# kit-cel/vae-equalizer

Measured on AMD Instinct MI355X. Metric: equalized symbols/s/GPU, DP 64-QAM VAE-LE, higher is better.
Workload: dtype f32

## Files before the change

vae_equalizer_amd/csrc/vaeq_dp_wave_kernel.h:

```cpp
#pragma once
#include <hip/hip_runtime.h>
#include <stdint.h>
#include <type_traits>

#include "vaeq.h"
#include "vaeq_common.h"
#include "vaeq_launch.h"
#include "vaeq_wave.h"

#ifdef VAEQ_PHASE_STAMPS
#define VAEQ_STAMP(i) do { if (s == a.steps - 1) tst[i] = __builtin_readcyclecounter(); } while (0)
#define VAEQ_XSTAMP(i) do { if (s == a.steps - 1) tsx[i] = __builtin_readcyclecounter(); } while (0)
#else
#define VAEQ_STAMP(i) do { } while (0)
#define VAEQ_XSTAMP(i) do { } while (0)
#endif
#define VAEQ_NSTAMP 12
#ifndef VAEQ_PIPE
#define VAEQ_PIPE 1
#endif
#define VAEQ_BT_FRAMES 16
#ifndef VAEQ_WPS
#define VAEQ_WPS 2
#endif

namespace vaeq {

__device__ __forceinline__ float half_sum(float a0, float a1)
{
    const auto r = __builtin_amdgcn_permlane32_swap(__builtin_bit_cast(unsigned, a0), __builtin_bit_cast(unsigned, a1), false, false);
    return __builtin_bit_cast(float, (unsigned)r[0]) + __builtin_bit_cast(float, (unsigned)r[1]);
}

struct WaveLayout {
    int Lph, Uph;
    int X, E, U, PSv, W, H, PSh, VS, MOM, RED, XG, total;
};

__host__ __device__ inline WaveLayout wave_layout(int B, int M, int NW = 1)
{
    WaveLayout l;
    const int len = 2 * B + M - 1;
    const int lph = wave_lph(len);
    l.Lph = lph;
    l.Uph = B / 2 + 1;
    int o = 0;
    auto take = [&](int bytes) { int r = o; o += (bytes + 15) & ~15; return r; };
    l.X = take(2 * 4 * lph * 8);
    l.E = take(2 * 4 * lph * 8);
    const int ubytes = 2 * 2 * l.Uph * 8, gbytes = 2 * B * 8;
    l.U = take(ubytes > gbytes ? ubytes : gbytes);
    l.PSv = take(2 * (B + 1) * 4);
    l.W = take(2 * M * 16);
    l.H = take(2 * 2 * (M + 1) * 8);
    l.PSh = take(2 * (M + 1) * 4);
    l.VS = take(2 * M * 4);
    l.MOM = take(16 * 64 * 4);
    l.RED = take(NW > 1 ? 64 * 4 : 0);
    l.XG = take((NW - 1) * 4 * 64 * 4);
    l.total = o;
    return l;
}

template <int M, bool INIT, bool PIPE = true, bool SPLIT = true>
__device__ __forceinline__ void pair_fir(cacc (&acc)[2][2], cacc (&accx)[2][2], const float2 *xp, int Lph, const float4 *wq)
{
    cacc (&acc2)[2][2] = SPLIT ? accx : acc;
    auto tapA = [&](int k) -> v2f { return lds2(reinterpret_cast<const float2 *>(wq + k)); };
    auto tapB = [&](int k) -> v2f { return lds2(reinterpret_cast<const float2 *>(wq + k) + 1); };
    constexpr int G = M / 4;
    auto load = [&](int g, v2f (&r)[14]) {
        const float2 *xg = xp + g;
        r[0] = lds2(xg); r[1] = lds2(xg + Lph); r[2] = lds2(xg + 2 * Lph); r[3] = lds2(xg + 3 * Lph); r[4] = lds2(xg + 1); r[5] = lds2(xg + Lph + 1);
#pragma unroll
        for (int t = 0; t < 4; t++) { r[6 + 2 * t] = tapA(4 * g + t); r[7 + 2 * t] = tapB(4 * g + t); }
    };
    auto fma = [&](int, const v2f (&r)[14], auto first) {
        constexpr bool F = decltype(first)::value;
        cmacf<F>(acc[0][0], r[6], r[0]); cmacf<F>(acc[0][1], r[7], r[0]); cmacf<F>(acc[1][0], r[6], r[2]); cmacf<F>(acc[1][1], r[7], r[2]);
        cmacf<F && SPLIT>(acc2[0][0], r[8], r[1]); cmacf<F && SPLIT>(acc2[0][1], r[9], r[1]);
        cmacf<F && SPLIT>(acc2[1][0], r[8], r[3]); cmacf<F && SPLIT>(acc2[1][1], r[9], r[3]);
        cmac(acc[0][0], r[10], r[2]); cmac(acc[0][1], r[11], r[2]); cmac(acc[1][0], r[10], r[4]); cmac(acc[1][1], r[11], r[4]);
        cmac(acc2[0][0], r[12], r[3]); cmac(acc2[0][1], r[13], r[3]); cmac(acc2[1][0], r[12], r[5]); cmac(acc2[1][1], r[13], r[5]);
    };
    pipe2<14, INIT, PIPE>(G, load, fma);
#pragma unroll
    for (int k = 4 * G; k < M; k++) {
        const v2f a = tapA(k), b = tapB(k);
        const v2f xa = lds2(xp + (k & 3) * Lph + (k >> 2)), xb = lds2(xp + ((k + 2) & 3) * Lph + ((k + 2) >> 2));
        if (k & 1) { cmac(acc2[0][0], a, xa); cmac(acc2[0][1], b, xa); cmac(acc2[1][0], a, xb); cmac(acc2[1][1], b, xb); }
        else { cmac(acc[0][0], a, xa); cmac(acc[0][1], b, xa); cmac(acc[1][0], a, xb); cmac(acc[1][1], b, xb); }
    }
}

template <int M, bool MERGE = true>
__device__ __forceinline__ void pair_du(cacc (&acc)[2][2][2], const float2 *ep, int Lph, const float2 *ht, int MP)
{
    constexpr int G = M / 4;
    auto load1 = [&](int chi, int g, v2f *x) {
        const float2 *xg = ep + chi * 4 * Lph + g;
        x[0] = lds2(xg); x[1] = lds2(xg + Lph); x[2] = lds2(xg + 2 * Lph); x[3] = lds2(xg + 3 * Lph); x[4] = lds2(xg + 1); x[5] = lds2(xg + Lph + 1);
#pragma unroll
        for (int t = 0; t < 4; t++) { x[6 + 2 * t] = lds2(ht + (chi * 2 + 0) * MP + 4 * g + t); x[7 + 2 * t] = lds2(ht + (chi * 2 + 1) * MP + 4 * g + t); }
    };
    auto fma1 = [&](int chi, const v2f *x, int t, auto first) {
        constexpr bool F = decltype(first)::value;
        cmacf<F>(acc[chi][0][0], x[6 + 2 * t], x[t]); cmacf<F>(acc[chi][0][1], x[7 + 2 * t], x[t]);
        cmacf<F>(acc[chi][1][0], x[6 + 2 * t], x[t + 2]); cmacf<F>(acc[chi][1][1], x[7 + 2 * t], x[t + 2]);
    };
    if constexpr (MERGE) {
        auto load = [&](int g, v2f (&r)[28]) { load1(0, g, r); load1(1, g, r + 14); };
        auto fma = [&](int, const v2f (&r)[28], auto first) {
            fma1(0, r, 0, first); fma1(1, r + 14, 0, first);
#pragma unroll
            for (int t = 1; t < 4; t++) { fma1(0, r, t, std::false_type{}); fma1(1, r + 14, t, std::false_type{}); }
        };
        pipe2<28, true, false>(G, load, fma);
    } else {
#pragma unroll
        for (int chi = 0; chi < 2; chi++) {
            auto load = [&](int g, v2f (&r)[14]) { load1(chi, g, r); };
            auto fma = [&](int, const v2f (&r)[14], auto first) {
                fma1(chi, r, 0, first);
#pragma unroll
                for (int t = 1; t < 4; t++) fma1(chi, r, t, std::false_type{});
            };
            pipe2<14, true, false>(G, load, fma);
        }
    }
#pragma unroll
    for (int k = 4 * G; k < M; k++)
#pragma unroll
        for (int chi = 0; chi < 2; chi++) {
            const float2 *xp = ep + chi * 4 * Lph;
            const v2f a = lds2(ht + (chi * 2 + 0) * MP + k), b = lds2(ht + (chi * 2 + 1) * MP + k);
            const v2f xa = lds2(xp + (k & 3) * Lph + (k >> 2)), xb = lds2(xp + ((k + 2) & 3) * Lph + ((k + 2) >> 2));
            cmac(acc[chi][0][0], a, xa); cmac(acc[chi][0][1], b, xa); cmac(acc[chi][1][0], a, xb); cmac(acc[chi][1][1], b, xb);
        }
}

constexpr bool uniform_parts(int B, int M, int NP)
{
    const int mh = M / 2, nm = 2 * B - 2 * mh;
    for (int par = 0; par < 2; par++) {
        const int T = (nm - par + 1) >> 1, Th = ((T + 2 * NP - 1) / (2 * NP)) << 1;
        int n0 = -1;
        for (int part = 0; part < NP; part++) {
            const int ma = (part * Th) >> 1, e = part * Th + Th, mb = ((T < e ? T : e) + 1) >> 1;
            if (mb - ma <= 0 || (n0 >= 0 && mb - ma != n0)) return false;
            n0 = mb - ma;
        }
    }
    const int Bq = ((B + 2 * NP - 1) / (2 * NP)) << 1;
    int n0 = -1;
    for (int part = 0; part < NP; part++) {
        const int ma = (part * Bq) >> 1, e = part * Bq + Bq, mb = (B < e ? B : e) >> 1;
        if (mb - ma <= 0 || (n0 >= 0 && mb - ma != n0)) return false;
        n0 = mb - ma;
    }
    return true;
}

template <int M, int NLEV, int BT, bool PAIR, int OUT, int NW = 1, int BL = 0>
__global__ __launch_bounds__(64 * NW, VAEQ_WPS) void dp_wave_kernel(const vaeq_dp_args a)
{
    constexpr int mh = M / 2, Mh = 2 * mh, MP = M + 1;
    constexpr float LOG2E = 1.4426950408889634f, LN2 = 0.6931471805599453f;
    extern __shared__ float4 smem4[];
    char *sm = reinterpret_cast<char *>(smem4);
    const int gl = threadIdx.x, lane = NW > 1 ? (gl & 63) : gl, wv = NW > 1 ? (gl >> 6) : 0, run = blockIdx.x;
    constexpr int NT = 64 * NW, NP = 2 * NW;
    constexpr bool UNI = BT > 0 && uniform_parts(BT, M, NP);
    constexpr bool FIXL = BT > 0 || (BL > 0 && M != 13 && M != 17 && !(M == 31 && NW == 1));
    constexpr bool PIPE = VAEQ_PIPE && FIXL;
    constexpr bool WIDE = FIXL;
    constexpr bool B100 = BT == 100 && NW == 1;
    constexpr int QAUX = B100 ? 2 : 0;
    const int B = BT ? BT : a.B;
    const int BS = BT ? BT : BL ? BL : B;
    constexpr bool ODDB = BT == 0 && BL > 0;
    const int L = 2 * B, nm = L - Mh, P2 = ODDB ? (B + 1) / 2 : B / 2;
    const float rnm = 1.0f / (float)nm;
    const WaveLayout lay = wave_layout(BS, M, NW);
    const int Lph = lay.Lph, Uph = lay.Uph;
    float2 *Xs = reinterpret_cast<float2 *>(sm + lay.X), *Es = reinterpret_cast<float2 *>(sm + lay.E);
    float2 *Us = reinterpret_cast<float2 *>(sm + lay.U), *GY = Us;
    float4 *Wt = reinterpret_cast<float4 *>(sm + lay.W);
    float2 *Ht = reinterpret_cast<float2 *>(sm + lay.H);
    float *PSv = reinterpret_cast<float *>(sm + lay.PSv);
    float *PSh = reinterpret_cast<float *>(sm + lay.PSh);
    float *VS = reinterpret_cast<float *>(sm + lay.VS);
    float *RED = reinterpret_cast<float *>(sm + lay.RED), *XG = reinterpret_cast<float *>(sm + lay.XG);

    float amp[NLEV], b2[NLEV], nlogP[NLEV];
    const float nusc = a.nu_sc[run];
#pragma unroll
    for (int i = 0; i < NLEV; i++) {
        amp[i] = a.amp[i];
        b2[i] = nusc * amp[i] * amp[i] * LOG2E;
        nlogP[i] = -logf(a.P[(size_t)run * NLEV + i]);
    }
    const float var0 = a.var[run * 2 + 0], var1 = a.var[run * 2 + 1];
    const float lrW = a.lr_W[run], lrH = a.lr_h[run];

    for (int i = gl; i < (lay.W - lay.X) / 8; i += NT) Xs[i] = make_float2(0.f, 0.f);
    for (int i = gl; i < (lay.PSh - lay.H) / 8; i += NT) Ht[i] = make_float2(0.f, 0.f);
    __syncthreads();
    const int tk = lane & 31, half = lane >> 5;
    const bool worker = tk < M, owner = worker && wv == 0;
    const int part = wv * 2 + half;
    const size_t gbase = (size_t)run * 8 * M;
    float *MOM = reinterpret_cast<float *>(sm + lay.MOM) + lane;
#define mWr(p) MOM[(0 + (p)) * 64]
#define mWi(p) MOM[(2 + (p)) * 64]
#define vWr(p) MOM[(4 + (p)) * 64]
#define vWi(p) MOM[(6 + (p)) * 64]
#define mHr(p) MOM[(8 + (p)) * 64]
#define mHi(p) MOM[(10 + (p)) * 64]
#define vHr(p) MOM[(12 + (p)) * 64]
#define vHi(p) MOM[(14 + (p)) * 64]
    if (owner) {
#pragma unroll
        for (int p = 0; p < 2; p++) {
            const size_t ir = gbase + (half * 4 + p) * M + tk, ii = gbase + (half * 4 + 2 + p) * M + tk;
            float *wq = reinterpret_cast<float *>(&Wt[p * M + tk]);
            wq[half * 2 + 0] = a.W[ir];
            wq[half * 2 + 1] = a.W[ii];
            mWr(p) = a.adam_mW[ir]; mWi(p) = a.adam_mW[ii];
            vWr(p) = a.adam_vW[ir]; vWi(p) = a.adam_vW[ii];
            const size_t hr = gbase + ((half * 2 + p) * 2 + 0) * M + tk, hi = hr + M;
            Ht[(half * 2 + p) * MP + tk] = make_float2(a.h[hr], a.h[hi]);
            mHr(p) = a.adam_mh[hr]; mHi(p) = a.adam_mh[hi];
            vHr(p) = a.adam_vh[hr]; vHi(p) = a.adam_vh[hi];
        }
    }
    int step = a.step[run];
    __shared__ double BTW[2][VAEQ_BT_FRAMES];
    if (gl < VAEQ_BT_FRAMES && gl < a.n_frames) {
        const double t = (double)(step + gl * a.steps);
        BTW[0][gl] = pow(0.9, t);
        BTW[1][gl] = pow(0.999, t);
    }
    __syncthreads();
    double b1t = BTW[0][0], b2t = BTW[1][0];

    const int klen = a.keep_len, k0 = a.keep_off;
    const size_t No = (size_t)a.steps * klen;
    constexpr bool pairst = PAIR;
    const bool act = gl < P2;
    const int nq = (nm + 3) / 4;
    const int n0 = 2 * gl;
    const bool v1 = ODDB ? act && (n0 + 1 < B) : act;
    const float2 *Xl = Xs + gl, *El = Es + gl, *Ul = Us + gl;
    const float2 *Xa = Xs + (act ? gl : 0), *Ea = Es + (act ? gl : 0);

    const bool ldl = gl < (ODDB ? (L + 3) / 4 : L / 4);
    float4 pf[4];
    const uint32_t S4 = (uint32_t)a.S * 4u;
    auto frame_rsrc = [&](int f) { return make_rsrc(a.rx + ((size_t)run * a.n_frames + f) * 4 * (size_t)a.S, 4u * S4); };
    auto fetch = [&](const __amdgpu_buffer_rsrc_t xr, int s) {
        const uint32_t vo = ldl ? ((uint32_t)s * (uint32_t)a.stride_sym * 2u + 4u * gl) * 4u : OOB;
#pragma unroll
        for (int r = 0; r < 4; r++) pf[r] = bld128(xr, vo, (uint32_t)r * S4);
    };
#ifdef VAEQ_PHASE_STAMPS
    long long tst[VAEQ_NSTAMP], tsx[8];
#endif
    fetch(frame_rsrc(0), 0);
    for (int f = 0; f < a.n_frames; f++) {
        const __amdgpu_buffer_rsrc_t xr = frame_rsrc(f), xn = frame_rsrc(f + 1 < a.n_frames ? f + 1 : f);
        if (f && f < VAEQ_BT_FRAMES) {
            b1t = BTW[0][f];
            b2t = BTW[1][f];
        }
        const bool qf = OUT != 2 && a.q_out, yf = a.y_out, ef = OUT != 1 && a.eq_out, df = OUT != 1 && a.dec_out;
        const uint32_t No4 = (uint32_t)No * 4u;
        const size_t fr = (size_t)run * a.n_frames + f;
        const __amdgpu_buffer_rsrc_t qr = make_rsrc(qf ? a.q_out + fr * (4 * NLEV) * No : nullptr, qf ? 4u * NLEV * No4 : 0u);
        const __amdgpu_buffer_rsrc_t yr = make_rsrc(yf ? a.y_out + fr * 4 * No : nullptr, yf ? 4u * No4 : 0u);
        const __amdgpu_buffer_rsrc_t er = make_rsrc(ef ? a.eq_out + fr * 2 * No : nullptr, ef ? 2u * No4 : 0u);
        const __amdgpu_buffer_rsrc_t dr = make_rsrc(df ? a.dec_out + fr * 4 * No : nullptr, df ? (uint32_t)(4 * No) : 0u);
        const __amdgpu_buffer_rsrc_t lr_ = make_rsrc(a.loss ? a.loss + fr * a.steps : nullptr, a.loss ? (uint32_t)a.steps * 4u : 0u);
        const __amdgpu_buffer_rsrc_t vr_ = make_rsrc(a.var_est ? a.var_est + fr * 2 * a.steps : nullptr, a.var_est ? (uint32_t)a.steps * 8u : 0u);
#pragma unroll 1
        for (int s = 0; s < a.steps; s++) {
            VAEQ_STAMP(0);
            if (ldl) {
#pragma unroll
                for (int p = 0; p < 2; p++) {
                    const float4 I4 = pf[p * 2 + 0], Q4 = pf[p * 2 + 1];
                    const float xi[4] = {I4.x, I4.y, I4.z, I4.w}, xq[4] = {Q4.x, Q4.y, Q4.z, Q4.w};
#pragma unroll
                    for (int i = 0; i < 4; i++) {
                        const int c = mh + i;
                        const bool in = !ODDB || 4 * gl + i < L;
                        Xs[(p * 4 + (c & 3)) * Lph + gl + (c >> 2)] = in ? make_float2(xi[i], xq[i]) : make_float2(0.f, 0.f);
                    }
                }
            }
            sync_lds<NW>();

            VAEQ_STAMP(1);
            float2 y[2][2];
            {
                cacc ya[2][2], yb[2][2];
                pair_fir<M, true, PIPE, WIDE>(ya, yb, Xa, Lph, Wt);
                pair_fir<M, false, PIPE, WIDE>(ya, yb, Xa + 4 * Lph, Lph, Wt + M);
#pragma unroll
                for (int sy = 0; sy < 2; sy++)
#pragma unroll
                    for (int o = 0; o < 2; o++) {
                        if constexpr (WIDE) {
                            ya[sy][o].a += yb[sy][o].a;
                            ya[sy][o].b += yb[sy][o].b;
                        }
                        y[sy][o] = cfin(ya[sy][o]);
                    }
            }
            asm volatile("" : "+v"(y[0][0].x), "+v"(y[0][0].y), "+v"(y[0][1].x), "+v"(y[0][1].y), "+v"(y[1][0].x), "+v"(y[1][0].y),
                         "+v"(y[1][1].x), "+v"(y[1][1].y));
            VAEQ_STAMP(2);
            const bool kept0 = act && (n0 >= k0) && (n0 < k0 + klen), kept1 = act && (n0 + 1 >= k0) && (n0 + 1 < k0 + klen);
            const uint32_t col = (uint32_t)(s * klen + (n0 - k0));
            const uint32_t vo0 = kept0 ? col * 4u : OOB, vo1 = kept1 ? col * 4u + 4u : OOB;
            if (yf) {
                uint32_t yrow = 0u;
                auto next_row = [&]() {
                    yrow += No4;
                    asm volatile("" : "+s"(yrow));
                };
#pragma unroll
                for (int o = 0; o < 2; o++) {
                    const uint32_t r0 = yrow;
                    next_row();
                    const uint32_t r1 = yrow;
                    next_row();
                    if (pairst) {
                        bst64(v2f{y[0][o].x, y[1][o].x}, yr, vo0, r0);
                        bst64(v2f{y[0][o].y, y[1][o].y}, yr, vo0, r1);
                    } else {
                        bst32(y[0][o].x, yr, vo0, r0); bst32(y[0][o].y, yr, vo0, r1);
                        bst32(y[1][o].x, yr, vo1, r0); bst32(y[1][o].y, yr, vo1, r1);
                    }
                }
            }

            VAEQ_STAMP(3);
            float mv[2][2][2], mt3[2][2][2], mkc[2][2][2];
            uint32_t qrow = 0u;
            float klsum = 0.f, vv[2][2];
#pragma unroll
            for (int o = 0; o < 2; o++) {
                const float c2 = 0.5f / (o ? var1 : var0) * LOG2E;
                float2 muv[2];
#pragma unroll
                for (int c = 0; c < 2; c++) {
                    const v2f yy = c ? v2f{y[0][o].y, y[1][o].y} : v2f{y[0][o].x, y[1][o].x};
                    v2f z[NLEV], q[NLEV];
                    v2f ssum = {0.f, 0.f};
                    float zm0 = -3.0e38f, zm1 = -3.0e38f;
#pragma unroll
                    for (int i = 0; i < NLEV; i++) {
                        const v2f d = yy - amp[i];
                        z[i] = -(d * d * c2 + b2[i]);
                        zm0 = fmaxf(zm0, z[i].x);
                        zm1 = fmaxf(zm1, z[i].y);
                    }
                    const v2f zmax = {zm0, zm1};
#pragma unroll
                    for (int i = 0; i < NLEV; i++) {
                        z[i] -= zmax;
                        q[i] = v2f{__builtin_amdgcn_exp2f(z[i].x), __builtin_amdgcn_exp2f(z[i].y)};
                        ssum += q[i];
                    }
                    const v2f rs = {__builtin_amdgcn_rcpf(ssum.x), __builtin_amdgcn_rcpf(ssum.y)};
                    v2f m1 = {0.f, 0.f};
#pragma unroll
                    for (int i = 0; i < NLEV; i++) {
                        q[i] *= rs;
                        m1 += q[i] * amp[i];
                    }
                    if (ef && c == 0) {
                        if (pairst) bst64(m1, er, vo0, (uint32_t)o * No4);
                        else { bst32(m1.x, er, vo0, (uint32_t)o * No4); bst32(m1.y, er, vo1, (uint32_t)o * No4); }
                    }
                    if (df) {
                        float v0 = q[0].x, v1 = q[0].y;
                        int b0 = 0, b1 = 0;
#pragma unroll
                        for (int i = 1; i < NLEV; i++) {
                            if (q[i].x > v0) { v0 = q[i].x; b0 = i; }
                            if (q[i].y > v1) { v1 = q[i].y; b1 = i; }
                        }
                        const uint32_t ro = (uint32_t)(o * 2 + c) * (uint32_t)No;
                        if (pairst) bst16((unsigned short)(b0 | (b1 << 8)), dr, kept0 ? col : OOB, ro);
                        else { bst8((unsigned char)b0, dr, kept0 ? col : OOB, ro); bst8((unsigned char)b1, dr, kept1 ? col + 1u : OOB, ro); }
                    }
                    v2f m2 = {0.f, 0.f}, m3 = {0.f, 0.f}, kk = {0.f, 0.f}, kl = {0.f, 0.f};
#pragma unroll
                    for (int i = 0; i < NLEV; i++) {
                        const v2f d = amp[i] - m1, qd = q[i] * d, g = z[i] * LN2 + nlogP[i];
                        m2 += qd * d;
                        m3 += qd * d * d;
                        kk += qd * g;
                        kl += q[i] * g;
                    }
                    const bool inr0 = (n0 >= mh) && (n0 < B - mh) && act;
                    const bool inr1 = (n0 + 1 >= mh) && (n0 + 1 < B - mh) && act;
                    if (inr0) klsum += kl.x - __builtin_amdgcn_logf(ssum.x) * LN2;
                    if (inr1) klsum += kl.y - __builtin_amdgcn_logf(ssum.y) * LN2;
                    asm volatile("" : "+v"(m2), "+v"(m3), "+v"(kk), "+v"(klsum));
                    mv[0][o][c] = m2.x; mv[1][o][c] = m2.y;
                    mt3[0][o][c] = m3.x; mt3[1][o][c] = m3.y;
                    mkc[0][o][c] = inr0 ? kk.x : 0.f;
                    mkc[1][o][c] = inr1 ? kk.y : 0.f;
                    if (c) { muv[0].y = m1.x; muv[1].y = m1.y; } else { muv[0].x = m1.x; muv[1].x = m1.y; }
                    if (qf) {
#pragma unroll
                        for (int i = 0; i < NLEV; i++) {
                            const uint32_t ro = qrow;
                            if (pairst) bst64<QAUX>(q[i], qr, vo0, ro);
                            else { bst32<QAUX>(q[i].x, qr, vo0, ro); bst32<QAUX>(q[i].y, qr, vo1, ro); }
                            qrow += No4;
                            asm volatile("" : "+s"(qrow));
                        }
                    }
                }
                vv[o][0] = act ? mv[0][o][0] + mv[0][o][1] : 0.f;
                vv[o][1] = v1 ? mv[1][o][0] + mv[1][o][1] : 0.f;
                if (act) {
                    Us[(o * 2 + 0) * Uph + gl] = muv[0];
                    Us[(o * 2 + 1) * Uph + gl] = v1 ? muv[1] : make_float2(0.f, 0.f);
                }
            }
            VAEQ_STAMP(4);
            {
                float inc[2];
#pragma unroll
                for (int o = 0; o < 2; o++) inc[o] = wave_incl_scan_dpp(vv[o][0] + vv[o][1]);
                if constexpr (NW > 1) {
                    if (lane == 63) { RED[wv] = inc[0]; RED[NW + wv] = inc[1]; }
                    sync_lds<NW>();
#pragma unroll
                    for (int w = 0; w < NW - 1; w++)
                        if (w < wv) { inc[0] += RED[w]; inc[1] += RED[NW + w]; }
                }
#pragma unroll
                for (int o = 0; o < 2; o++) {
                    if (act) {
                        PSv[o * (BS + 1) + n0 + 1] = inc[o] - vv[o][1];
                        PSv[o * (BS + 1) + n0 + 2] = inc[o];
                    }
                    if (gl == 0) PSv[o * (BS + 1)] = 0.f;
                }
            }
            sync_lds<NW>();
            if (owner) {
                const int lo = (Mh - tk + 1) >> 1, hi_ = (nm - 1 + Mh - tk) >> 1;
                VS[half * M + tk] = PSv[half * (BS + 1) + hi_ + 1] - PSv[half * (BS + 1) + lo];
            }
            sync_lds<NW>();

            VAEQ_STAMP(5);
            float se0 = 0.f, se1 = 0.f;
            float hq0 = 0.f, hq1 = 0.f;
            if (worker) {
                const float2 h0 = Ht[(0 * 2 + half) * MP + tk], h1 = Ht[(1 * 2 + half) * MP + tk];
                hq0 = h0.x * h0.x + h0.y * h0.y;
                hq1 = h1.x * h1.x + h1.y * h1.y;
            }
            const float vsl = worker ? VS[half * M + tk] : 0.f;
            {
                cacc D[2][4];
                constexpr int NA = mh + 1, NB = NA / 2;
#pragma unroll
                for (int v = 0; v < 2; v++) {
                    const float2 *h0 = Ht + (0 * 2 + v) * MP, *h1 = Ht + (1 * 2 + v) * MP;
                    const float2 *up = Us + (gl < nq ? gl : 0) + v * 2 * Uph;
                    auto step_a = [&](int aa, v2f ulo, v2f uhi, auto first) {
                        constexpr bool F = decltype(first)::value;
                        const v2f e0 = lds2(h0 + 2 * aa), o0 = lds2(h0 + 2 * aa + 1), e1 = lds2(h1 + 2 * aa), o1 = lds2(h1 + 2 * aa + 1);
                        cmacf<F>(D[0][0], e0, ulo); cmacf<F>(D[0][1], o0, ulo);
                        cmacf<F>(D[0][2], e0, uhi); cmacf<F>(D[0][3], o0, uhi);
                        cmacf<F>(D[1][0], e1, ulo); cmacf<F>(D[1][1], o1, ulo);
                        cmacf<F>(D[1][2], e1, uhi); cmacf<F>(D[1][3], o1, uhi);
                    };
                    if (NA & 1) {
                        if (v == 0) step_a(mh, lds2(up), lds2(up + Uph), std::true_type{});
                        else step_a(mh, lds2(up), lds2(up + Uph), std::false_type{});
                    } else if (v == 0) {
#pragma unroll
                        for (int chi = 0; chi < 2; chi++)
#pragma unroll
                            for (int i = 0; i < 4; i++) D[chi][i] = cacc0();
                    }
                    constexpr int ph = mh & 1;
                    auto load = [&](int b, v2f (&r)[11]) {
                        const int sl = (mh >> 1) - b;
                        r[0] = lds2(up + ph * Uph + sl);
                        r[1] = lds2(up + (ph ^ 1) * Uph + sl + ph);
                        r[2] = lds2(up + (ph ^ 1) * Uph + sl + ph - 1);
#pragma unroll
                        for (int t = 0; t < 4; t++) { r[3 + t] = lds2(h0 + 4 * b + t); r[7 + t] = lds2(h1 + 4 * b + t); }
                    };
                    auto fma = [&](int, const v2f (&r)[11], auto) {
                        cmac(D[0][0], r[3], r[0]); cmac(D[0][1], r[4], r[0]); cmac(D[0][2], r[3], r[1]); cmac(D[0][3], r[4], r[1]);
                        cmac(D[1][0], r[7], r[0]); cmac(D[1][1], r[8], r[0]); cmac(D[1][2], r[7], r[1]); cmac(D[1][3], r[8], r[1]);
                        cmac(D[0][0], r[5], r[2]); cmac(D[0][1], r[6], r[2]); cmac(D[0][2], r[5], r[0]); cmac(D[0][3], r[6], r[0]);
                        cmac(D[1][0], r[9], r[2]); cmac(D[1][1], r[10], r[2]); cmac(D[1][2], r[9], r[0]); cmac(D[1][3], r[10], r[0]);
                    };
                    pipe2<11, false, PIPE>(NB, load, fma);
                }
                VAEQ_STAMP(6);
                if (gl < nq) {
#pragma unroll
                    for (int chi = 0; chi < 2; chi++)
#pragma unroll
                        for (int i = 0; i < 4; i++) {
                            const int ce = Mh + i;
                            const float2 x = Xl[(chi * 4 + (ce & 3)) * Lph + (ce >> 2)];
                            const float2 Dv = cfin(D[chi][i]);
                            float2 e = make_float2(x.x - Dv.x, x.y - Dv.y);
                            if (4 * gl + i >= nm) e = make_float2(0.f, 0.f);
                            Es[(chi * 4 + (ce & 3)) * Lph + gl + (ce >> 2)] = e;
                            const float e2 = e.x * e.x + e.y * e.y;
                            if (chi) se1 += e2; else se0 += e2;
                        }
                }
            }
            se0 = wave_sum_dpp(se0);
            se1 = wave_sum_dpp(se1);
            klsum = wave_sum_dpp(klsum);
            if constexpr (NW > 1) {
                if (lane == 0) { RED[16 + wv] = se0; RED[16 + NW + wv] = se1; RED[16 + 2 * NW + wv] = klsum; }
                sync_lds<NW>();
                se0 = RED[16]; se1 = RED[16 + NW]; klsum = RED[16 + 2 * NW];
#pragma unroll
                for (int w = 1; w < NW; w++) { se0 += RED[16 + w]; se1 += RED[16 + NW + w]; klsum += RED[16 + 2 * NW + w]; }
            }
            const float C0 = se0 + wave_sum_dpp(hq0 * vsl), C1 = se1 + wave_sum_dpp(hq1 * vsl);
            const float gC0 = (float)nm * __builtin_amdgcn_rcpf(C0), gC1 = (float)nm * __builtin_amdgcn_rcpf(C1);
            {
                const uint32_t vo = gl == 0 ? 0u : OOB;
                if (a.loss) bst32((float)nm * LN2 * (__builtin_amdgcn_logf(C0) + __builtin_amdgcn_logf(C1)) + klsum, lr_, vo, (uint32_t)s * 4u);
                if (a.var_est) {
                    bst32(C0 * rnm, vr_, vo, (uint32_t)s * 4u);
                    bst32(C1 * rnm, vr_, vo, ((uint32_t)a.steps + (uint32_t)s) * 4u);
                }
            }
            {
                const float inc = half_incl_scan_dpp(gC0 * hq0 + gC1 * hq1);
                if (owner) PSh[half * MP + tk + 1] = inc;
                if (tk == 0) PSh[half * MP] = 0.f;
            }
            sync_lds<NW>();

            VAEQ_STAMP(7);
            step += 1;
            b1t *= 0.9;
            b2t *= 0.999;
            const float rbc1 = __builtin_amdgcn_rcpf((float)(1.0 - b1t));
            const float bc2s = __builtin_amdgcn_rcpf(__builtin_amdgcn_sqrtf((float)(1.0 - b2t)));
            const float ssW = lrW * rbc1, ssH = lrH * rbc1;
            float2 hnew[2];
            hnew[0] = hnew[1] = make_float2(0.f, 0.f);
            float ghr[2] = {0, 0}, ghi[2] = {0, 0};
            float2 hacc[2];
            {
                float2 ph_h[2] = {make_float2(0.f, 0.f), make_float2(0.f, 0.f)};
                float ph_vs[2] = {0.f, 0.f};
                if (NW == 1 && owner) {
#pragma unroll
                    for (int v = 0; v < 2; v++) {
                        ph_h[v] = Ht[(half * 2 + v) * MP + tk];
                        ph_vs[v] = VS[v * M + tk];
                    }
                }
                cacc ca[2][2];
                {
                    const int tkc = worker ? tk : 0, par = tkc & 1, aa = tkc >> 1;
                    const int T = (nm - par + 1) >> 1, Th = ((T + 2 * NP - 1) / (2 * NP)) << 1;
                    const int ma = (part * Th) >> 1, mb = (min(T, part * Th + Th) + 1) >> 1;
                    const int ceA = par + Mh, ceB = par + Mh + 2, npA = mh - aa, npB = mh - aa + 1;
                    const float2 *eA = Es + (ceA & 3) * Lph + (ceA >> 2) + ma, *eB = Es + (ceB & 3) * Lph + (ceB >> 2) + ma;
                    const float2 *uA = Us + (npA & 1) * Uph + (npA >> 1) + ma, *uB = Us + (npB & 1) * Uph + (npB >> 1) + ma;
                    auto load1 = [&](int m, v2f *r) {
                        r[0] = lds2(eA + m); r[1] = lds2(eA + 4 * Lph + m); r[2] = lds2(uA + m); r[3] = lds2(uA + 2 * Uph + m);
                        r[4] = lds2(eB + m); r[5] = lds2(eB + 4 * Lph + m); r[6] = lds2(uB + m); r[7] = lds2(uB + 2 * Uph + m);
                    };
                    cacc cbx[2][2];
                    cacc (&cb)[2][2] = WIDE ? cbx : ca;
                    auto fma1 = [&](const v2f *r, auto first) {
                        constexpr bool F = decltype(first)::value;
                        cmacf<F>(ca[0][0], r[2], r[0]); cmacf<F>(ca[0][1], r[3], r[0]); cmacf<F>(ca[1][0], r[2], r[1]); cmacf<F>(ca[1][1], r[3], r[1]);
                        cmacf<F && WIDE>(cb[0][0], r[6], r[4]); cmacf<F && WIDE>(cb[0][1], r[7], r[4]); cmacf<F && WIDE>(cb[1][0], r[6], r[5]); cmacf<F && WIDE>(cb[1][1], r[7], r[5]);
                    };
                    auto load = [&](int i, v2f (&r)[16]) { load1(2 * i, r); load1(2 * i + 1, r + 8); };
                    auto fma = [&](int, const v2f (&r)[16], auto first) { fma1(r, first); fma1(r + 8, std::false_type{}); };
                    int n = mb - ma;
                    VAEQ_XSTAMP(0);
                    if constexpr (UNI) {
                        n = __builtin_amdgcn_readfirstlane(n);
                        pipe2<16, true, PIPE>(n >> 1, load, fma);
                    } else {
                        ca[0][0] = ca[0][1] = ca[1][0] = ca[1][1] = cbx[0][0] = cbx[0][1] = cbx[1][0] = cbx[1][1] = cacc0();
                        pipe2<16, false, PIPE>(n >> 1, load, fma);
                    }
                    if (n & 1) {
                        v2f r[8];
                        load1(n - 1, r);
                        fma1(r, std::false_type{});
                    }
                    if constexpr (WIDE) {
#pragma unroll
                        for (int i = 0; i < 2; i++)
#pragma unroll
                            for (int j = 0; j < 2; j++) { ca[i][j].a += cbx[i][j].a; ca[i][j].b += cbx[i][j].b; }
                    }
                }
                VAEQ_XSTAMP(1);
                float2 acc[2][2];
#pragma unroll
                for (int chi = 0; chi < 2; chi++)
#pragma unroll
                    for (int v = 0; v < 2; v++) acc[chi][v] = cfinc(ca[chi][v]);
                if constexpr (B100) {
#pragma unroll
                    for (int v = 0; v < 2; v++) {
                        acc[0][v].x = acc[1][v].x = half_sum(acc[0][v].x, acc[1][v].x);
                        acc[0][v].y = acc[1][v].y = half_sum(acc[0][v].y, acc[1][v].y);
                    }
                } else {
#pragma unroll
                    for (int chi = 0; chi < 2; chi++)
#pragma unroll
                        for (int v = 0; v < 2; v++) {
                            acc[chi][v].x += __shfl_xor(acc[chi][v].x, 32, 64);
                            acc[chi][v].y += __shfl_xor(acc[chi][v].y, 32, 64);
                        }
                }
                if constexpr (NW > 1) {
#pragma unroll
                    for (int v = 0; v < 2; v++) {
                        hacc[v] = half ? acc[1][v] : acc[0][v];
                        if (wv > 0) {
                            XG[((wv - 1) * 4 + 2 * v + 0) * 64 + lane] = hacc[v].x;
                            XG[((wv - 1) * 4 + 2 * v + 1) * 64 + lane] = hacc[v].y;
                        }
                    }
                }
                VAEQ_XSTAMP(2);
                if (NW == 1 && owner) {
                    const float g = half ? gC1 : gC0;
#pragma unroll
                    for (int v = 0; v < 2; v++) {
                        const float2 ac = half ? acc[1][v] : acc[0][v];
                        const float2 hh = ph_h[v];
                        const float vs = ph_vs[v];
                        ghr[v] = g * (-2.0f * ac.x + 2.0f * hh.x * vs);
                        ghi[v] = g * (-2.0f * ac.y + 2.0f * hh.y * vs);
                        hnew[v] = hh;
                        if (!a.no_update) {
                            adam_update_fast(hnew[v].x, mHr(v), vHr(v), ghr[v], ssH, bc2s);
                            adam_update_fast(hnew[v].y, mHi(v), vHi(v), ghi[v], ssH, bc2s);
                        }
                    }
                }
            }

            asm volatile("" : "+v"(hnew[0].x), "+v"(hnew[0].y), "+v"(hnew[1].x), "+v"(hnew[1].y), "+v"(ghr[0]), "+v"(ghr[1]), "+v"(ghi[0]),
                         "+v"(ghi[1]));
            {
                const bool last_s = s + 1 == a.steps;
                if constexpr (B100) {
                    const bool more = !(last_s && f + 1 == a.n_frames);
                    const uint32_t vo = ldl && more ? ((uint32_t)(last_s ? 0 : s + 1) * (uint32_t)a.stride_sym * 2u + 4u * gl) * 4u : OOB;
#pragma unroll
                    for (int r = 0; r < 4; r++) pf[r] = bld128(last_s ? xn : xr, vo, (uint32_t)r * S4);
                } else if (!(last_s && f + 1 == a.n_frames)) fetch(last_s ? xn : xr, last_s ? 0 : s + 1);
            }
            VAEQ_XSTAMP(3);
            VAEQ_STAMP(8);
            float2 gy[2][2];
            {
                float2 au0[2][2], au1[2][2];
                {
                    cacc cu[2][2][2];
                    pair_du<M, WIDE>(cu, Ea, Lph, Ht, MP);
#pragma unroll
                    for (int sy = 0; sy < 2; sy++)
#pragma unroll
                        for (int v = 0; v < 2; v++) { au0[sy][v] = cfinc(cu[0][sy][v]); au1[sy][v] = cfinc(cu[1][sy][v]); }
                }
#pragma unroll
                for (int sy = 0; sy < 2; sy++) {
                    const int sx = 2 * (n0 + sy);
                    const int jlo = max(0, Mh - sx), jhi = max(jlo - 1, min(Mh, nm - 1 + Mh - sx));
#pragma unroll
                    for (int v = 0; v < 2; v++) {
                        const float ur = -2.0f * (gC0 * au0[sy][v].x + gC1 * au1[sy][v].x);
                        const float ui = -2.0f * (gC0 * au0[sy][v].y + gC1 * au1[sy][v].y);
                        const float gv = PSh[v * MP + jhi + 1] - PSh[v * MP + jlo];
                        const float iv = 1.0f / (v ? var1 : var0);
                        gy[sy][v].x = iv * (ur * mv[sy][v][0] + gv * mt3[sy][v][0] + mkc[sy][v][0]);
                        gy[sy][v].y = iv * (ui * mv[sy][v][1] + gv * mt3[sy][v][1] + mkc[sy][v][1]);
                    }
                }
            }
            VAEQ_STAMP(9);
            sync_lds<NW>();
            if constexpr (NW > 1) {
                if (owner) {
                    const float g = half ? gC1 : gC0;
#pragma unroll
                    for (int v = 0; v < 2; v++) {
                        float2 ac = hacc[v];
#pragma unroll
                        for (int w = 0; w < NW - 1; w++) {
                            ac.x += XG[(w * 4 + 2 * v + 0) * 64 + lane];
                            ac.y += XG[(w * 4 + 2 * v + 1) * 64 + lane];
                        }
                        const float2 hh = Ht[(half * 2 + v) * MP + tk];
                        const float vs = VS[v * M + tk];
                        ghr[v] = g * (-2.0f * ac.x + 2.0f * hh.x * vs);
                        ghi[v] = g * (-2.0f * ac.y + 2.0f * hh.y * vs);
                        hnew[v] = hh;
                        if (!a.no_update) {
                            adam_update_fast(hnew[v].x, mHr(v), vHr(v), ghr[v], ssH, bc2s);
                            adam_update_fast(hnew[v].y, mHi(v), vHi(v), ghi[v], ssH, bc2s);
                        }
                    }
                }
            }
            if (act) {
#pragma unroll
                for (int v = 0; v < 2; v++) {
                    GY[v * BS + n0] = gy[0][v];
                    GY[v * BS + n0 + 1] = v1 ? gy[1][v] : make_float2(0.f, 0.f);
                }
            }
            if (owner && !a.no_update) {
                Ht[(half * 2 + 0) * MP + tk] = hnew[0];
                Ht[(half * 2 + 1) * MP + tk] = hnew[1];
            }
            sync_lds<NW>();

            VAEQ_STAMP(10);
            float gwr[2] = {0, 0}, gwi[2] = {0, 0};
            {
                float pw_w[2][2] = {{0.f, 0.f}, {0.f, 0.f}}, pw_m[2][2] = {{0.f, 0.f}, {0.f, 0.f}}, pw_v[2][2] = {{0.f, 0.f}, {0.f, 0.f}};
                if (owner) {
#pragma unroll
                    for (int p = 0; p < 2; p++) {
                        const float *wq = reinterpret_cast<const float *>(&Wt[p * M + tk]) + half * 2;
                        pw_w[p][0] = wq[0]; pw_w[p][1] = wq[1];
                        pw_m[p][0] = mWr(p); pw_m[p][1] = mWi(p);
                        pw_v[p][0] = vWr(p); pw_v[p][1] = vWi(p);
                    }
                }
                cacc ca[2][2];
                {
                    const int tkc = worker ? tk : 0;
                    const int Be = ODDB ? B + (B & 1) : B;
                    const int Bq = ((Be + 2 * NP - 1) / (2 * NP)) << 1;
                    const int ma = (part * Bq) >> 1, mb = min(Be, part * Bq + Bq) >> 1;
                    const int cA = tkc, cB = tkc + 2;
                    const float2 *xA = Xs + (cA & 3) * Lph + (cA >> 2) + ma, *xB = Xs + (cB & 3) * Lph + (cB >> 2) + ma;
                    const float2 *G0 = GY + 2 * ma, *G1 = GY + BS + 2 * ma;
                    auto load1 = [&](int m, v2f *r) {
                        r[0] = lds2(G0 + 2 * m); r[1] = lds2(G0 + 2 * m + 1); r[2] = lds2(G1 + 2 * m); r[3] = lds2(G1 + 2 * m + 1);
                        r[4] = lds2(xA + m); r[5] = lds2(xA + 4 * Lph + m); r[6] = lds2(xB + m); r[7] = lds2(xB + 4 * Lph + m);
                    };
                    cacc cbx[2][2];
                    cacc (&cb)[2][2] = WIDE ? cbx : ca;
                    auto fma1 = [&](const v2f *r, auto first) {
                        constexpr bool F = decltype(first)::value;
                        cmacf<F>(ca[0][0], r[4], r[0]); cmacf<F>(ca[0][1], r[5], r[0]); cmacf<F>(ca[1][0], r[4], r[2]); cmacf<F>(ca[1][1], r[5], r[2]);
                        cmacf<F && WIDE>(cb[0][0], r[6], r[1]); cmacf<F && WIDE>(cb[0][1], r[7], r[1]); cmacf<F && WIDE>(cb[1][0], r[6], r[3]); cmacf<F && WIDE>(cb[1][1], r[7], r[3]);
                    };
                    auto load = [&](int i, v2f (&r)[16]) { load1(2 * i, r); load1(2 * i + 1, r + 8); };
                    auto fma = [&](int, const v2f (&r)[16], auto first) { fma1(r, first); fma1(r + 8, std::false_type{}); };
                    int n = mb - ma;
                    VAEQ_XSTAMP(4);
                    if constexpr (UNI) {
                        n = __builtin_amdgcn_readfirstlane(n);
                        pipe2<16, true, PIPE>(n >> 1, load, fma);
                    } else {
                        ca[0][0] = ca[0][1] = ca[1][0] = ca[1][1] = cbx[0][0] = cbx[0][1] = cbx[1][0] = cbx[1][1] = cacc0();
                        pipe2<16, false, PIPE>(n >> 1, load, fma);
                    }
                    if (n & 1) {
                        v2f r[8];
                        load1(n - 1, r);
                        fma1(r, std::false_type{});
                    }
                    if constexpr (WIDE) {
#pragma unroll
                        for (int i = 0; i < 2; i++)
#pragma unroll
                            for (int j = 0; j < 2; j++) { ca[i][j].a += cbx[i][j].a; ca[i][j].b += cbx[i][j].b; }
                    }
                }
                VAEQ_XSTAMP(5);
                float2 acc[2][2];
#pragma unroll
                for (int o = 0; o < 2; o++)
#pragma unroll
                    for (int pp = 0; pp < 2; pp++) acc[o][pp] = cfinc(ca[o][pp]);
                if constexpr (B100) {
#pragma unroll
                    for (int p = 0; p < 2; p++) {
                        acc[0][p].x = acc[1][p].x = half_sum(acc[0][p].x, acc[1][p].x);
                        acc[0][p].y = acc[1][p].y = half_sum(acc[0][p].y, acc[1][p].y);
                    }
                } else {
#pragma unroll
                    for (int o = 0; o < 2; o++)
#pragma unroll
                        for (int p = 0; p < 2; p++) {
                            acc[o][p].x += __shfl_xor(acc[o][p].x, 32, 64);
                            acc[o][p].y += __shfl_xor(acc[o][p].y, 32, 64);
                        }
                }
                if constexpr (NW > 1) {
#pragma unroll
                    for (int p = 0; p < 2; p++) {
                        const float2 ac = half ? acc[1][p] : acc[0][p];
                        if (wv > 0) {
                            XG[((wv - 1) * 4 + 2 * p + 0) * 64 + lane] = ac.x;
                            XG[((wv - 1) * 4 + 2 * p + 1) * 64 + lane] = ac.y;
                        }
                    }
                    sync_lds<NW>();
                }
                VAEQ_XSTAMP(6);
                if (owner) {
#pragma unroll
                    for (int p = 0; p < 2; p++) {
                        float2 ac = half ? acc[1][p] : acc[0][p];
                        if constexpr (NW > 1) {
#pragma unroll
                            for (int w = 0; w < NW - 1; w++) {
                                ac.x += XG[(w * 4 + 2 * p + 0) * 64 + lane];
                                ac.y += XG[(w * 4 + 2 * p + 1) * 64 + lane];
                            }
                        }
                        gwr[p] = ac.x;
                        gwi[p] = ac.y;
                        if (!a.no_update) {
                            float *wq = reinterpret_cast<float *>(&Wt[p * M + tk]) + half * 2;
                            float wr = pw_w[p][0], wi = pw_w[p][1];
                            adam_update_fast(wr, pw_m[p][0], pw_v[p][0], gwr[p], ssW, bc2s);
                            adam_update_fast(wi, pw_m[p][1], pw_v[p][1], gwi[p], ssW, bc2s);
                            wq[0] = wr;
                            wq[1] = wi;
                            mWr(p) = pw_m[p][0]; mWi(p) = pw_m[p][1];
                            vWr(p) = pw_v[p][0]; vWi(p) = pw_v[p][1];
                        }
                    }
                }
            }
            if (a.dbg_gW && owner && f == a.n_frames - 1 && s == a.steps - 1) {
#pragma unroll
                for (int p = 0; p < 2; p++) {
                    a.dbg_gW[gbase + (half * 4 + p) * M + tk] = gwr[p];
                    a.dbg_gW[gbase + (half * 4 + 2 + p) * M + tk] = gwi[p];
                    a.dbg_gh[gbase + ((half * 2 + p) * 2 + 0) * M + tk] = ghr[p];
                    a.dbg_gh[gbase + ((half * 2 + p) * 2 + 1) * M + tk] = ghi[p];
                }
            }
            sync_lds<NW>();
            VAEQ_XSTAMP(7);
            VAEQ_STAMP(11);
        }
    }
#ifdef VAEQ_PHASE_STAMPS
    if (gl == 0 && run == (int)gridDim.x / 2 && a.loss)
        for (int i = 0; i + 1 < VAEQ_NSTAMP; i++) a.loss[i] = (float)(tst[i + 1] - tst[i]);
    if (gl == 0 && run == (int)gridDim.x / 2 && a.loss)
        for (int i = 0; i < 7; i++) a.loss[16 + i] = (float)(tsx[i + 1] - tsx[i]);
#endif

    if (owner && !a.no_update) {
#pragma unroll
        for (int p = 0; p < 2; p++) {
            const size_t ir = gbase + (half * 4 + p) * M + tk, ii = gbase + (half * 4 + 2 + p) * M + tk;
            const float *wq = reinterpret_cast<const float *>(&Wt[p * M + tk]) + half * 2;
            a.W[ir] = wq[0]; a.W[ii] = wq[1];
            a.adam_mW[ir] = mWr(p); a.adam_mW[ii] = mWi(p);
            a.adam_vW[ir] = vWr(p); a.adam_vW[ii] = vWi(p);
            const size_t hr = gbase + ((half * 2 + p) * 2 + 0) * M + tk, hi = hr + M;
            const float2 hh = Ht[(half * 2 + p) * MP + tk];
            a.h[hr] = hh.x; a.h[hi] = hh.y;
            a.adam_mh[hr] = mHr(p); a.adam_mh[hi] = mHi(p);
            a.adam_vh[hr] = vHr(p); a.adam_vh[hi] = vHi(p);
        }
    }
    if (gl == 0 && !a.no_update) a.step[run] = step;
#undef mWr
#undef mWi
#undef vWr
#undef vWi
#undef mHr
#undef mHi
#undef vHr
#undef vHi
}


template <int M, int NLEV, int BT, int NW, int BL, bool SPEC>
static int launch_wave(const vaeq_dp_args &a, hipStream_t st)
{
    const size_t lds = (size_t)wave_layout(BL ? BL : a.B, M, NW).total;
    const bool pair = ((a.keep_len | a.keep_off) & 1) == 0;
    const int out = !SPEC ? 0 : (!a.eq_out && !a.dec_out) ? 1 : !a.q_out ? 2 : 0;
    constexpr int O1 = SPEC ? 1 : 0, O2 = SPEC ? 2 : 0;
    void (*const k[2][3])(const vaeq_dp_args) = {
        {dp_wave_kernel<M, NLEV, BT, false, 0, NW, BL>, dp_wave_kernel<M, NLEV, BT, false, O1, NW, BL>, dp_wave_kernel<M, NLEV, BT, false, O2, NW, BL>},
        {dp_wave_kernel<M, NLEV, BT, true, 0, NW, BL>, dp_wave_kernel<M, NLEV, BT, true, O1, NW, BL>, dp_wave_kernel<M, NLEV, BT, true, O2, NW, BL>}};
    note_kernel("vaeq::dp_wave_kernel<%d, %d, %d, %s, %d, %d, %d>", M, NLEV, BT, pair ? "true" : "false", out, NW, BL);
    return launch(k[pair][out], dim3(a.R), dim3(64 * NW), lds, st, a);
}

template <int M, int NLEV, int BT, int NW, int BL>
static int64_t wave_resident(int B)
{
    int nb = 0, dev = 0;
    hipDeviceProp_t prop;
    if (hipGetDevice(&dev) != hipSuccess || hipGetDeviceProperties(&prop, dev) != hipSuccess) return VAEQ_ERR_DEVICE;
    auto k = dp_wave_kernel<M, NLEV, BT, true, 0, NW, BL>;
    if (hipOccupancyMaxActiveBlocksPerMultiprocessor(&nb, k, 64 * NW, (size_t)wave_layout(BL ? BL : B, M, NW).total) != hipSuccess) return VAEQ_ERR_DEVICE;
    return (int64_t)nb * prop.multiProcessorCount;
}

template <int M, int BT, int NW>
static int launch_wave_lev(const vaeq_dp_args &a, hipStream_t st)
{
    return dispatch_nlev(a.n_lev, [&](auto nl) { return launch_wave<M, decltype(nl)::value, BT, NW, 0, (BT > 0)>(a, st); });
}
template <int M, int BT, int NW>
static int64_t wave_resident_lev(int B, int n_lev)
{
    return dispatch_nlev(n_lev, [&](auto nl) { return wave_resident<M, decltype(nl)::value, BT, NW, 0>(B); });
}
template <int M, int BL, int NW, bool SPEC>
static int launch_wave_fixl_lev(const vaeq_dp_args &a, hipStream_t st)
{
    return dispatch_nlev(a.n_lev, [&](auto nl) { return launch_wave<M, decltype(nl)::value, 0, NW, BL, SPEC>(a, st); });
}
template <int M, int BL, int NW>
static int64_t wave_resident_fixl_lev(int n_lev)
{
    return dispatch_nlev(n_lev, [&](auto nl) { return wave_resident<M, decltype(nl)::value, 0, NW, BL>(BL); });
}

template <int NW>
static int launch_wave_any(const vaeq_dp_args &a, hipStream_t st)
{
    switch (a.M) {
    case 25: return launch_wave_lev<25, 0, NW>(a, st);
    case 31: return launch_wave_fixl_lev<31, 128 * NW, NW, false>(a, st);
    case 21: return launch_wave_fixl_lev<21, 128 * NW, NW, false>(a, st);
    case 17: return launch_wave_fixl_lev<17, 128 * NW, NW, false>(a, st);
    case 13: return launch_wave_fixl_lev<13, 128 * NW, NW, false>(a, st);
    case 9: return launch_wave_fixl_lev<9, 128 * NW, NW, false>(a, st);
    }
    return VAEQ_ERR_SHAPE;
}

template <int NW>
static int64_t wave_resident_any(int B, int M, int n_lev)
{
    switch (M) {
    case 25: return wave_resident_lev<25, 0, NW>(B, n_lev);
    case 31: return wave_resident_fixl_lev<31, 128 * NW, NW>(n_lev);
    case 21: return wave_resident_fixl_lev<21, 128 * NW, NW>(n_lev);
    case 17: return wave_resident_fixl_lev<17, 128 * NW, NW>(n_lev);
    case 13: return wave_resident_fixl_lev<13, 128 * NW, NW>(n_lev);
    case 9: return wave_resident_fixl_lev<9, 128 * NW, NW>(n_lev);
    }
    return VAEQ_ERR_SHAPE;
}

}
```

Baseline: 10.52 billion.

## Map three output taus per lane in B=100 M=25 DP conv-error stage

Adds a specialized path for B=100, M=25 in which each lane computes three consecutive output positions for one polarization, with a compile-time check that the mapping covers every tau exactly once. Channel taps are loaded once and reused across the three outputs, and loads are software-pipelined. Error values go to LDS and are then re-read to form the squared-error sums. The intent is to reduce redundant LDS loads and idle lanes compared with the generic two-output mapping, at the cost of more registers and extra code complexity.

New measurement: 10.78 billion, median of 6. 1.02x the previous value.

```diff
diff --git a/vae_equalizer_amd/csrc/vaeq_dp_wave_kernel.h b/vae_equalizer_amd/csrc/vaeq_dp_wave_kernel.h
--- a/vae_equalizer_amd/csrc/vaeq_dp_wave_kernel.h
+++ b/vae_equalizer_amd/csrc/vaeq_dp_wave_kernel.h
@@ -160,6 +160,35 @@
     }
     return true;
 }
+
+struct D3Map {
+    static constexpr int TPL = 3;
+    static constexpr int nm_lanes(int T) { return (T + TPL - 1) / TPL; }
+    static constexpr int chi(int lane) { return lane >> 5; }
+    static constexpr bool works(int lane, int T) { return (lane & 31) < nm_lanes(T); }
+    static constexpr int m(int lane, int T) { return works(lane, T) ? (lane & 31) : 0; }
+    static constexpr bool stores(int lane, int i, int T) { return works(lane, T) && TPL * m(lane, T) + i < T; }
+    static constexpr bool exact(int B, int M)
+    {
+        const int mh = M / 2, T = B - mh, Uph = B / 2 + 1;
+        if (nm_lanes(T) > 32 || T > 128) return false;
+        for (int c = 0; c < 2; c++) {
+            int cnt[128] = {};
+            for (int lane = 0; lane < 64; lane++)
+                for (int i = 0; i < TPL; i++) {
+                    const int tau = TPL * m(lane, T) + i;
+                    if (tau + mh >= 2 * Uph) return false;
+                    if (chi(lane) != c || !stores(lane, i, T)) continue;
+                    if (tau >= T) return false;
+                    cnt[tau]++;
+                }
+            for (int tau = 0; tau < 128; tau++)
+                if (cnt[tau] != (tau < T ? 1 : 0)) return false;
+        }
+        return true;
+    }
+};
+static_assert(D3Map::exact(100, 25), "B = 100: three tau per lane must cover tau = 0..87 of both chi exactly once");
 
 template <int M, int NLEV, int BT, bool PAIR, int OUT, int NW = 1, int BL = 0>
 __global__ __launch_bounds__(64 * NW, VAEQ_WPS) void dp_wave_kernel(const vaeq_dp_args a)
@@ -470,7 +499,94 @@
                 hq1 = h1.x * h1.x + h1.y * h1.y;
             }
             const float vsl = worker ? VS[half * M + tk] : 0.f;
-            {
+            if constexpr (B100 && M == 25) {
+                constexpr int T = 100 - mh, NB = (mh + 1) / 2;
+                static_assert((mh & 1) == 0 && (Mh & 3) == 0 && D3Map::exact(100, M), "D3Map: mh even (a = mh stands alone, its odd tap is the pad)");
+                int l3 = lane;
+                asm volatile("" : "+v"(l3));
+                const int m3 = D3Map::m(l3, T), modd = m3 & 1, m3h = (3 * m3) >> 1;
+                cacc D3[3][2];
+                const int xo = D3Map::chi(l3) * 4 * Lph + (Mh >> 2) + m3h;
+                const int o0 = xo + (modd ? 2 * Lph : 0), o2 = xo + (modd ? 1 : 2 * Lph);
+                const int off[6] = {o0, o0 + Lph, o2, o2 + Lph, o0 + 1, o0 + Lph + 1};
+                v2f x6[6];
+#pragma unroll
+                for (int k = 0; k < 6; k++) x6[k] = lds2(Xs + off[k]);
+                {
+                    const float2 *uE = Us + modd * Uph + m3h, *uO = Us + (modd ^ 1) * Uph + m3h + modd;
+                    const float2 *hc = Ht + D3Map::chi(l3) * 2 * MP;
+                    v2f am[2][4];
+#pragma unroll
+                    for (int v = 0; v < 2; v++) {
+                        am[v][0] = lds2(hc + v * MP + Mh);
+                        am[v][1] = lds2(uE + v * 2 * Uph); am[v][2] = lds2(uO + v * 2 * Uph); am[v][3] = lds2(uE + v * 2 * Uph + 1);
+                    }
+#pragma unroll
+                    for (int v = 0; v < 2; v++) {
+                        const float2 *hv = hc + v * MP, *ue = uE + v * 2 * Uph, *uo = uO + v * 2 * Uph;
+                        {
+                            const v2f t = am[v][0], u0 = am[v][1], u1 = am[v][2], u2 = am[v][3];
+                            if (v == 0) { cmul(D3[0][0], t, u0); cmul(D3[1][0], t, u1); cmul(D3[2][0], t, u2); }
+                            else { cmac(D3[0][0], t, u0); cmac(D3[1][0], t, u1); cmac(D3[2][0], t, u2); }
+                        }
+                        auto load = [&](int b, v2f (&r)[8]) {
+                            const int sl = (mh >> 1) - b;
+                            r[0] = lds2(uo + sl - 1); r[1] = lds2(ue + sl); r[2] = lds2(uo + sl); r[3] = lds2(ue + sl + 1);
+#pragma unroll
+                            for (int t = 0; t < 4; t++) r[4 + t] = lds2(hv + 4 * b + t);
+                        };
+                        auto fma = [&](int, const v2f (&r)[8], auto first) {
+                            constexpr bool F = decltype(first)::value;
+                            v2f t0 = r[4], t1 = r[5], t2 = r[6], t3 = r[7];
+                            asm volatile("" : "+v"(t0), "+v"(t1));
+#pragma unroll
+                            for (int i = 0; i < 3; i++) {
+                                cmac(D3[i][0], t0, r[i + 1]);
+                                cmacf<F>(D3[i][1], t1, r[i + 1]);
+                                if constexpr (F) asm volatile("" : "+v"(D3[i][1].a), "+v"(D3[i][1].b));
+                            }
+                            asm volatile("" : "+v"(t2), "+v"(t3));
+#pragma unroll
+                            for (int i = 0; i < 3; i++) { cmac(D3[i][0], t2, r[i]); cmac(D3[i][1], t3, r[i]); }
+                        };
+                        if (v == 0) pipe2<8, true, PIPE>(NB, load, fma);
+                        else pipe2<8, false, PIPE>(NB, load, fma);
+                    }
+                }
+                VAEQ_STAMP(6);
+                {
+                    float2 e[6];
+#pragma unroll
+                    for (int k = 0; k < 6; k++) {
+                        const float2 x = f2(x6[k]);
+                        const float2 Dv = cfin(D3[k >> 1][k & 1]);
+                        e[k] = make_float2(x.x - Dv.x, x.y - Dv.y);
+                        if (6 * (D3Map::nm_lanes(T) - 1) + k >= 2 * T && 6 * m3 + k >= nm) e[k] = make_float2(0.f, 0.f);
+                    }
+                    if (D3Map::works(l3, T)) {
+#pragma unroll
+                        for (int k = 0; k < 6; k++) Es[off[k]] = e[k];
+                    }
+                }
+                sync_lds<NW>();
+                {
+                    const float2 *Eq = Es + (gl < nq ? gl : 0);
+                    v2f eq[2][4];
+#pragma unroll
+                    for (int chi = 0; chi < 2; chi++)
+#pragma unroll
+                        for (int i = 0; i < 4; i++) eq[chi][i] = lds2(Eq + (chi * 4 + ((Mh + i) & 3)) * Lph + ((Mh + i) >> 2));
+#pragma unroll
+                    for (int chi = 0; chi < 2; chi++)
+#pragma unroll
+                        for (int i = 0; i < 4; i++) {
+                            const float2 e = f2(eq[chi][i]);
+                            const float e2 = __builtin_fmaf(e.x, e.x, e.y * e.y);
+                            if (chi) se1 += e2; else se0 += e2;
+                        }
+                    if (gl >= nq) se0 = se1 = 0.f;
+                }
+            } else {
                 cacc D[2][4];
                 constexpr int NA = mh + 1, NB = NA / 2;
 #pragma unroll
```
